# IannLiu/ReactRanker

Measured on AMD Instinct MI355X. Metric: queries/sec (lists scored+loss) ListMLE, higher is better.
Workload: dtype f32; 1 GPU; ListMLE 100k queries x 64 candidates (BASELINE.json configs[2]), 64-query steps, D-MPNN depth=3 hidden=300; preset=mle64, phase=train step: fwd + loss + bwd + grad all-reduce + Adam/NoamLR, candidates_per_query=64, pad_width_K=4, step_pool=6, parallelism=dp1

## Files before the change

include/reactranker_hip.h:

```cpp
#ifndef REACTRANKER_HIP_H
#define REACTRANKER_HIP_H

#include <stddef.h>
#include <stdint.h>

#ifdef __cplusplus
extern "C" {
#endif

typedef void* rr_stream_t;

typedef enum rr_status {
  RR_OK = 0,
  RR_ERR_ARG = -1,
  RR_ERR_ALIGN = -2,
  RR_ERR_LAUNCH = -3,
  RR_ERR_UNSUPPORTED = -4,
  RR_ERR_WORKSPACE = -5
} rr_status;

const char* rr_strerror(int status);
int rr_version(void);
void rr_abi_struct_sizes(size_t* linear_args, size_t* wgrad_args);
size_t rr_abi_gather_epi_size(void);
// ... 7 lines not shown
                             const int32_t* idx, int64_t n_out, int K, int H,
                             const float* row0_partial, int64_t n_partial, int64_t ld_partial,
                             float* out, int64_t ld_out, rr_stream_t stream);
int rr_gather_sum_amax_f32(const float* src, int64_t n_src, int64_t ld_src, const int32_t* idx, int64_t n_out, int K,
                           int H, const float* row0_partial, int64_t n_partial, int64_t ld_partial, float* out,
                           int64_t ld_out, float* amax_out, rr_stream_t stream);

int rr_gather_sum_masked_f32(const float* src, const float* mask, int64_t n_src, int64_t ld_src,
                             const int32_t* idx, int64_t n_out, int K, int H, float scale,
                             float* out, int64_t ld_out, rr_stream_t stream);
int rr_gather_sum_dropmask_f32(const float* src, int64_t n_src, int64_t ld_src, const float* y, int64_t ld_y,
                               const int32_t* idx, int64_t n_out, int K, int H, float drop_p, uint64_t drop_seed,
                               float scale, float* out, int64_t ld_out, rr_stream_t stream);

int rr_gather2_sum_dropmask_f32(const float* src, int64_t n_src, int64_t ld_src, const int32_t* in_idx, int64_t n_mid, int Ki,
                                const float* row0_partial, int64_t n_partial, int64_t ld_partial,
                                const float* y, int64_t ld_y, const int32_t* out_idx, int64_t n_out, int Ko, int H,
                                float drop_p, uint64_t drop_seed, float scale, float* out, int64_t ld_out,
                                rr_stream_t stream);

int rr_gather_sum_dropsrc_f32(const float* y, int64_t n_y, int64_t ld_y, const int32_t* map, int64_t n_map,
                              const int32_t* idx, int64_t n_out, int K, int H, float drop_p, uint64_t drop_seed,
                              float* out, int64_t ld_out, rr_stream_t stream);

#define RR_MAX_GATHER_SRCS 4
int rr_gather_sum_multi_f32(const float* const* srcs, int n_srcs, int64_t n_src, int64_t ld_src,
                            const int32_t* idx, int64_t n_out, int K, int H,
                            float* out, int64_t ld_out, rr_stream_t stream);

#define RR_MAX_GATHER_ADDS 15
typedef struct rr_gather_epi {
  const float* mask;        int64_t ld_mask;
  const uint8_t* mask_bits;
  float mask_scale;
  int n_adds;               int64_t ld_add;
  const float* adds[RR_MAX_GATHER_ADDS];
  float* amax_out;
} rr_gather_epi;
int rr_gather_sum_epi_f32(const float* src, int64_t n_src, int64_t ld_src,
                          const int32_t* idx, int64_t n_out, int K, int H,
                          const float* row0_partial, int64_t n_partial, int64_t ld_partial,
                          const rr_gather_epi* epi, float* out, int64_t ld_out, rr_stream_t stream);

int rr_gather_sum_csr_f32(const float* src, int64_t n_src, int64_t ld_src,
                          const int32_t* offsets, const int32_t* idx, int64_t n_out, int H,
                          float* out, int64_t ld_out, rr_stream_t stream);
// ... 558 lines not shown
```

reactranker_amd/_lib.py:

```python
from __future__ import annotations

import ctypes as C
import os

import torch

_HERE = os.path.dirname(os.path.abspath(__file__))
LIB_PATH = os.environ.get("RR_LIB_PATH") or os.path.join(_HERE, "csrc", "libreactranker_hip.so")

c_f32p = C.c_void_p
c_i32p = C.c_void_p
c_stream = C.c_void_p
i64 = C.c_int64
i32 = C.c_int
u64 = C.c_uint64
f32 = C.c_float


class LinearArgs(C.Structure):
    _fields_ = [
        ("M", i64), ("N", i32),
        ("a1", c_f32p), ("lda1", i64), ("k1", i32), ("a1_idx", c_i32p),
        ("a1_sub", c_f32p), ("lda1_sub", i64), ("a1_sub_idx", c_i32p),
        ("a2", c_f32p), ("lda2", i64), ("k2", i32),
# ... 134 lines not shown

_SIGS = {
    "rr_strerror": (C.c_char_p, [i32]),
    "rr_version": (i32, []),
    "rr_lds_opt_ins": (C.c_longlong, []),
    "rr_abi_struct_sizes": (None, [C.POINTER(C.c_size_t), C.POINTER(C.c_size_t)]),
    "rr_gather_sum_f32": (i32, [c_f32p, i64, i64, c_i32p, i64, i32, i32, c_f32p, i64, c_stream]),
    "rr_abi_gather_epi_size": (C.c_size_t, []),
    "rr_gather_sum_epi_f32": (i32, [c_f32p, i64, i64, c_i32p, i64, i32, i32, c_f32p, i64, i64, C.POINTER(GatherEpi), c_f32p, i64,
                                    c_stream]),
    "rr_segment_mean_bwd_masked_f32": (i32, [c_f32p, i64, c_i32p, c_i32p, i64, i32, i32, f32, u64, c_f32p, i64, C.c_void_p, f32,
                                             c_f32p, i64, c_stream]),
    "rr_segment_mean_bwd_masked_amax_f32": (i32, [c_f32p, i64, c_i32p, c_i32p, i64, i32, i32, f32, u64, c_f32p, i64, C.c_void_p, f32,
                                             c_f32p, i64, c_f32p, c_stream]),
    "rr_gather_sum_masked_f32": (i32, [c_f32p, c_f32p, i64, i64, c_i32p, i64, i32, i32, f32, c_f32p, i64, c_stream]),
    "rr_gather_sum_dropmask_f32": (i32, [c_f32p, i64, i64, c_f32p, i64, c_i32p, i64, i32, i32, f32, u64, f32, c_f32p, i64, c_stream]),
    "rr_gather2_sum_dropmask_f32": (i32, [c_f32p, i64, i64, c_i32p, i64, i32, c_f32p, i64, i64, c_f32p, i64, c_i32p, i64, i32, i32,
                                          f32, u64, f32, c_f32p, i64, c_stream]),
    "rr_gather_sum_dropsrc_f32": (i32, [c_f32p, i64, i64, c_i32p, i64, c_i32p, i64, i32, i32, f32, u64, c_f32p, i64, c_stream]),
    "rr_gather_sum_csr_f32": (i32, [c_f32p, i64, i64, c_i32p, c_i32p, i64, i32, c_f32p, i64, c_stream]),
    "rr_build_fbonds_f32": (i32, [c_f32p, i64, i64, i32, c_i32p, c_f32p, i64, i32, i64, c_f32p, i64, c_stream]),
    "rr_gather_diff_f32": (i32, [c_f32p, i64, i64, c_i32p, c_f32p, i64, i64, c_i32p, i64, i32, c_f32p, i64, c_stream]),
    "rr_gather_dropout_f32": (i32, [c_f32p, i64, i64, c_i32p, i64, i32, f32, u64, c_f32p, i64, c_stream]),
    "rr_gather_dropout_amax_f32": (i32, [c_f32p, i64, i64, c_i32p, i64, i32, f32, u64, c_f32p, i64, c_f32p, c_stream]),
    "rr_colsum_workspace_bytes": (C.c_size_t, [i64, i32]),
    "rr_weighted_colsum_f32": (i32, [c_f32p, i64, i64, c_f32p, i32, c_f32p, i32, C.c_void_p, C.c_size_t, c_stream]),
    "rr_linear_f32": (i32, [C.POINTER(LinearArgs), c_stream]),
    "rr_linear_colsum_rows": (i64, [i64]),
    "rr_linear_split_tail_launches": (i64, []),
    "rr_gather_sum_multi_f32": (i32, [C.POINTER(C.c_void_p), i32, i64, i64, c_i32p, i64, i32, i32, c_f32p, i64, c_stream]),
    "rr_gather_sum_padrow_f32": (i32, [c_f32p, i64, i64, c_i32p, i64, i32, i32, c_f32p, i64, i64, c_f32p, i64, c_stream]),
    "rr_gather_sum_amax_f32": (i32, [c_f32p, i64, i64, c_i32p, i64, i32, i32, c_f32p, i64, i64, c_f32p, i64, c_f32p, c_stream]),
    "rr_packed_weight_ld": (i64, [i32, i32]),
    "rr_mask_bits_row_bytes": (i64, [i32]),
    "rr_split_weight_bytes": (C.c_size_t, [i32, i32, i32]),
    "rr_pack_weight_f32": (i32, [c_f32p, i64, i32, i32, i32, i32, i32, c_f32p, c_stream]),
    "rr_pack_weights_f32": (i32, [C.c_void_p, i32, c_stream]),
    "rr_linear_wgrad_workspace_bytes": (C.c_size_t, [i64, i32, i32]),
    "rr_linear_wgrad_f32": (i32, [C.POINTER(WgradArgs), c_stream]),
    "rr_amax_f32": (i32, [c_f32p, i64, i32, i64, c_f32p, c_stream]),
    "rr_dropout_keep_host": (i32, [u64, u64, f32]),
    "rr_dropout_f32": (i32, [c_f32p, i64, f32, u64, c_f32p, c_stream]),
    "rr_relu_bwd_f32": (i32, [c_f32p, c_f32p, f32, c_f32p, c_f32p, i64, c_stream]),
    "rr_relu_bwd_sum_f32": (i32, [c_f32p, c_f32p, f32, C.POINTER(C.c_void_p), i32, c_f32p, i64, c_stream]),
    "rr_axpby_f32": (i32, [f32, c_f32p, f32, c_f32p, c_f32p, i64, c_stream]),
    "rr_head_fwd_f32": (i32, [c_f32p, i64, i32, i32, c_f32p, c_stream]),
# ... 218 lines not shown
```

reactranker_amd/csrc/gather.hip:

```cpp
#include "rr_common.h"
#include <initializer_list>

namespace {

template <int VEC> struct Vec;
template <> struct Vec<4> { using T = f32x4; };
template <> struct Vec<1> { using T = float; };

template <int VEC>
__device__ inline typename Vec<VEC>::T ld(const float* p) {
  return *reinterpret_cast<const typename Vec<VEC>::T*>(p);
}
template <int VEC>
__device__ inline void st(float* p, typename Vec<VEC>::T v) {
  *reinterpret_cast<typename Vec<VEC>::T*>(p) = v;
}

__device__ __attribute__((aligned(16))) const float gather_zero[4] = {0.f, 0.f, 0.f, 0.f};

template <int VEC>
__device__ __forceinline__ typename Vec<VEC>::T ld_row(const float* src, int64_t ld_src, int32_t j, int c) {
  return ld<VEC>(j >= 0 ? src + j * ld_src + c : gather_zero);
}

// ... 372 lines not shown
      for (int t = 0; t < Ko; ++t) {
        const int32_t j = orow[t];
        f32x4 inner = f32x4(0.0f);
        if (j >= 0) inner = gather_plain_sum<4>(A.src, A.ld_src, A.in_idx + static_cast<int64_t>(j) * Ki, Ki, c);
        acc = acc + dropmask_term(A, j, c, yv, inner);
      }
    }
    st<4>(A.out + r * A.ld_out + c, acc);
  }
}

struct DropSrc {
  const float* y;          int64_t ld_y;
  const int32_t* map;
  const int32_t* idx;      int64_t n_out; int K;
  int HV, H;
  uint32_t thr; float keep_scale; uint64_t seed;
  float* out;              int64_t ld_out;
};
__device__ __forceinline__ f32x4 dropsrc_term(const DropSrc& A, int32_t j, int c, f32x4 v) {
  if (A.thr != 0u) v = keep_scale4(v, A.seed, static_cast<uint64_t>(j < 0 ? 0 : j) * static_cast<uint64_t>(A.H) + static_cast<uint64_t>(c), A.thr, A.keep_scale);
  return v;
}
template <int KT>
__global__ void __launch_bounds__(256) gather_sum_dropsrc_kernel(const DropSrc A) {
  const int HV = A.HV, K = A.K;
  const int64_t total = A.n_out * HV;
#ifdef RR_GATHER_WALK
  if constexpr (KT > 0) {
    int64_t beg, end;
    gather_block_range(static_cast<int>(gridDim.x), total, &beg, &end);
    int64_t e = beg + threadIdx.x;
    if (e >= end) return;
    const int quo = 256 / HV, rem = 256 - quo * HV;
    int64_t r = e / HV;
    int q = static_cast<int>(e - r * HV);
    auto next = [&](int64_t& rr, int& qq) {
      rr += quo;
      qq += rem;
      if (qq >= HV) {
        qq -= HV;
        ++rr;
      }
    };
    auto maps = [&](const int32_t (&jj)[KT], int32_t (&mm)[KT]) {
#pragma unroll
      for (int k = 0; k < KT; ++k) mm[k] = A.map[jj[k] < 0 ? 0 : jj[k]];
    };
    int64_t r1 = r;
    int q1 = q;
    next(r1, q1);
    bool has1 = e + 256 < end;
    int32_t j[KT], m[KT], j1[KT], m1[KT], j2[KT];
#pragma unroll
    for (int k = 0; k < KT; ++k) j[k] = A.idx[r * KT + k];
#pragma unroll
    for (int k = 0; k < KT; ++k) j1[k] = A.idx[(has1 ? r1 : r) * KT + k];
    maps(j, m);
    while (true) {
      int64_t r2 = r1;
      int q2 = q1;
      next(r2, q2);
      const bool has2 = e + 512 < end;
#pragma unroll
      for (int k = 0; k < KT; ++k) j2[k] = A.idx[(has2 ? r2 : r) * KT + k];
      maps(j1, m1);
      const int c = q * 4;
      f32x4 v[KT];
#pragma unroll
      for (int k = 0; k < KT; ++k) v[k] = ld<4>(A.y + static_cast<int64_t>((j[k] < 0 || m[k] < 0) ? 0 : m[k]) * A.ld_y + c);
      f32x4 acc = f32x4(0.0f);
#pragma unroll
      for (int k = 0; k < KT; ++k) {
        f32x4 t = f32x4(0.0f);
        if (j[k] >= 0 && m[k] >= 0) t = dropsrc_term(A, j[k], c, v[k]);
        acc = acc + t;
      }
      st<4>(A.out + r * A.ld_out + c, acc);
      if (!has1) break;
      e += 256;
      r = r1;
      q = q1;
      r1 = r2;
      q1 = q2;
      has1 = has2;
#pragma unroll
      for (int k = 0; k < KT; ++k) {
        j[k] = j1[k];
        m[k] = m1[k];
        j1[k] = j2[k];
      }
    }
    return;
  }
#endif
  RR_GATHER_LOOP(e, static_cast<int>(gridDim.x), total) {
    const int64_t r = e / HV;
    const int c = static_cast<int>(e - r * HV) * 4;
    const f32x4 acc = gather_row_sum<f32x4>(
        A.idx + r * K, K,
        [&](int32_t j) { return ld_row<4>(A.y, A.ld_y, *(j >= 0 ? A.map + j : gather_none), c); },
        [&](int32_t j, f32x4 v) { return dropsrc_term(A, j, c, v); });
    st<4>(A.out + r * A.ld_out + c, acc);
  }
}

constexpr int GMAX = RR_MAX_GATHER_ADDS;
struct GatherEpi {
  const float* mask;   int64_t ld_mask;
  const uint8_t* bits; int64_t bits_row;
  float scale;
  int n_adds;          int64_t ld_add;
  const float* adds[GMAX];
  float* amax_out;
};

__device__ inline uint32_t epi_nibble(const uint8_t* bits, int64_t bits_row, int64_t r, int c) {
  const int blk = c / 304, cc = c - blk * 304;
  const uint32_t b = bits[r * bits_row + blk * 40 + ((cc & 15) >> 3) * 20 + (cc >> 4)];
  return (b >> (cc & 4)) & 0xFu;
}

template <int NADD>
struct EpiAux {
  uint32_t nib;
  f32x4 m;
  f32x4 a[NADD > 0 ? NADD : 1];
// ... 281 lines not shown
__global__ void __launch_bounds__(256) segment_mean_bwd_kernel(const float* __restrict__ dout, int64_t ld_dout,
                                                               const int32_t* __restrict__ a_scope,
                                                               const int32_t* __restrict__ atom2mol, int64_t n_atoms,
                                                               int H, int F, uint32_t thr, float keep_scale,
                                                               uint64_t seed, float* __restrict__ dx, int64_t ldx) {
  const int64_t total = n_atoms * H;
  const int64_t stride = static_cast<int64_t>(gridDim.x) * blockDim.x;
  const int W = H + F;
  for (int64_t e = static_cast<int64_t>(blockIdx.x) * blockDim.x + threadIdx.x; e < total; e += stride) {
    const int64_t a = e / H;
    const int c = static_cast<int>(e - a * H);
    const int32_t m = atom2mol[a];
    float v = 0.f;
    if (m >= 0) {
      const int32_t size = a_scope[2 * static_cast<int64_t>(m) + 1];
      v = dout[static_cast<int64_t>(m) * ld_dout + c] / static_cast<float>(size);
      if (thr != 0u)
        v = rr_keep(seed, static_cast<uint64_t>(m) * W + c, thr) ? v * keep_scale : 0.f;
    }
    dx[a * ldx + c] = v;
  }
}

__global__ void __launch_bounds__(256) segment_mean_bwd_vec_kernel(const float* __restrict__ dout, int64_t ld_dout,
                                                                   const int32_t* __restrict__ a_scope,
                                                                   const int32_t* __restrict__ atom2mol, int64_t n_atoms,
                                                                   int HV, int W, uint32_t thr, float keep_scale,
                                                                   uint64_t seed, float* __restrict__ dx, int64_t ldx,
                                                                   const float* __restrict__ mask, int64_t ld_mask,
                                                                   const uint8_t* __restrict__ mask_bits, int64_t bits_row,
                                                                   float mask_scale, float* __restrict__ amax_out) {
  const int64_t total = n_atoms * HV;
  const int64_t stride = static_cast<int64_t>(gridDim.x) * blockDim.x;
  float am = 0.f;
  for (int64_t e = static_cast<int64_t>(blockIdx.x) * blockDim.x + threadIdx.x; e < total; e += stride) {
    const int64_t a = e / HV;
    const int c = static_cast<int>(e - a * HV) * 4;
    const int32_t m = atom2mol[a];
    float4 v = make_float4(0.f, 0.f, 0.f, 0.f);
    if (m >= 0) {
      const float size = static_cast<float>(a_scope[2 * static_cast<int64_t>(m) + 1]);
      const float* d = dout + static_cast<int64_t>(m) * ld_dout + c;
      v = make_float4(d[0] / size, d[1] / size, d[2] / size, d[3] / size);
      if (thr != 0u) {
        const uint64_t i0 = static_cast<uint64_t>(m) * W + c;
        const uint32_t w0 = rr_hash_group(seed, i0 >> 2);
        const uint32_t w1 = (i0 & 3u) ? rr_hash_group(seed, (i0 >> 2) + 1) : w0;
        float* pv = &v.x;
#pragma unroll
        for (int k = 0; k < 4; ++k) {
          const uint64_t i = i0 + k;
          const uint32_t w = (i >> 2) == (i0 >> 2) ? w0 : w1;
          pv[k] = rr_hash_lane(w, static_cast<uint32_t>(i) & 3u) >= thr ? pv[k] * keep_scale : 0.f;
        }
      }
    }
    if (mask_bits != nullptr) v = mask_select(v, epi_nibble(mask_bits, bits_row, a, c), mask_scale);
    else if (mask != nullptr) v = mask_select(v, ld<4>(mask + a * ld_mask + c), mask_scale);
    *reinterpret_cast<float4*>(dx + a * ldx + c) = v;
    am = fmaxf(fmaxf(am, fmaxf(fabsf(v.x), fabsf(v.y))), fmaxf(fabsf(v.z), fabsf(v.w)));
  }
  amax_commit(am, amax_out);
}

bool rows_are_chunks(int H, std::initializer_list<int64_t> lds, std::initializer_list<const void*> ptrs) {
  bool ok = H % 4 == 0;
  for (const int64_t ld : lds) ok = ok && ld % 4 == 0;
  for (const void* p : ptrs) ok = ok && rr_aligned16(p);
  return ok;
}

#define RR_LAUNCH_ROWS(vec, kernel, n_out, H, pad_blocks, s, ...)                                       \
  do {                                                                                                  \
    if (vec) {                                                                                          \
      const int W = (H) / 4;                                                                            \
      kernel<4><<<rr_grid_for((n_out) * W, 256) + ((pad_blocks) ? W : 0), 256, 0, s>>>(__VA_ARGS__);    \
    } else {                                                                                            \
      const int W = (H);                                                                                \
      kernel<1><<<rr_grid_for((n_out) * W, 256) + ((pad_blocks) ? W : 0), 256, 0, s>>>(__VA_ARGS__);    \
    }                                                                                                   \
  } while (0)

}

extern "C" {

int rr_gather_sum_amax_f32(const float* src, int64_t n_src, int64_t ld_src, const int32_t* idx, int64_t n_out, int K,
                           int H, const float* row0_partial, int64_t n_partial, int64_t ld_partial, float* out,
                           int64_t ld_out, float* amax_out, rr_stream_t stream) {
  RR_CHECK_ARG(src && idx && out && n_src >= 0 && n_out >= 0 && K >= 1 && H >= 1 && ld_src >= H && ld_out >= H);
  RR_CHECK_ARG(!row0_partial || (n_out >= 1 && n_partial >= 0 && ld_partial >= H));
  if (n_out == 0) return RR_OK;
  hipStream_t s = static_cast<hipStream_t>(stream);
  bool vec = rows_are_chunks(H, {ld_src, ld_out}, {src, out});
  if (row0_partial) vec = vec && rows_are_chunks(H, {ld_partial}, {row0_partial});
  RR_LAUNCH_ROWS(vec, gather_sum_kernel, n_out, H, row0_partial != nullptr, s, src, ld_src, idx, n_out, K, W, out, ld_out,
                 row0_partial, n_partial, ld_partial, amax_out);
  return rr_launch_status();
}

int rr_gather_sum_f32(const float* src, int64_t n_src, int64_t ld_src, const int32_t* idx, int64_t n_out, int K,
                      int H, float* out, int64_t ld_out, rr_stream_t stream) {
  return rr_gather_sum_amax_f32(src, n_src, ld_src, idx, n_out, K, H, nullptr, 0, 0, out, ld_out, nullptr, stream);
}
// ... 132 lines not shown
  RR_CHECK_ARG(drop_p >= 0.f && drop_p < 1.f);
  if (!rows_are_chunks(H, {ld_y, ld_out}, {y, out})) return RR_ERR_ALIGN;
  if (n_out == 0) return RR_OK;
  DropSrc A;
  A.y = y; A.ld_y = ld_y; A.map = map; A.idx = idx; A.n_out = n_out; A.K = K; A.HV = H / 4; A.H = H;
  A.thr = rr_drop_threshold(drop_p); A.keep_scale = 1.0f / (1.0f - drop_p); A.seed = drop_seed; A.out = out; A.ld_out = ld_out;
  hipStream_t s = static_cast<hipStream_t>(stream);
  if (n_map == 0 || n_y == 0) {
    if (hipMemset2DAsync(out, static_cast<size_t>(ld_out) * sizeof(float), 0, static_cast<size_t>(H) * sizeof(float),
                         static_cast<size_t>(n_out), s) != hipSuccess) return RR_ERR_LAUNCH;
    return RR_OK;
  }
  const int grid = rr_grid_for(n_out * A.HV, 256);
  switch (K) {
    case 1: gather_sum_dropsrc_kernel<1><<<grid, 256, 0, s>>>(A); break;
    case 2: gather_sum_dropsrc_kernel<2><<<grid, 256, 0, s>>>(A); break;
    case 3: gather_sum_dropsrc_kernel<3><<<grid, 256, 0, s>>>(A); break;
    case 4: gather_sum_dropsrc_kernel<4><<<grid, 256, 0, s>>>(A); break;
    default: gather_sum_dropsrc_kernel<0><<<grid, 256, 0, s>>>(A); break;
  }
  return rr_launch_status();
}

int rr_gather_sum_csr_f32(const float* src, int64_t n_src, int64_t ld_src, const int32_t* offsets, const int32_t* idx,
                          int64_t n_out, int H, float* out, int64_t ld_out, rr_stream_t stream) {
  RR_CHECK_ARG(src && offsets && out && n_src >= 0 && n_out >= 0 && H >= 1 && ld_src >= H && ld_out >= H);
  if (n_out == 0) return RR_OK;
  hipStream_t s = static_cast<hipStream_t>(stream);
  const bool vec = rows_are_chunks(H, {ld_src, ld_out}, {src, out});
  RR_LAUNCH_ROWS(vec, gather_sum_csr_kernel, n_out, H, false, s, src, ld_src, offsets, idx, n_out, W, out, ld_out);
  return rr_launch_status();
}

int rr_gather_diff_f32(const float* a, int64_t n_a, int64_t ld_a, const int32_t* ia, const float* m, int64_t n_m,
                       int64_t ld_m, const int32_t* im, int64_t n_out, int H, float* out, int64_t ld_out,
                       rr_stream_t stream) {
  RR_CHECK_ARG(a && ia && m && im && out && n_a >= 0 && n_m >= 0 && n_out >= 0 && H >= 1 && ld_a >= H &&
               ld_m >= H && ld_out >= H);
  if (n_out == 0) return RR_OK;
  hipStream_t s = static_cast<hipStream_t>(stream);
  const bool vec = rows_are_chunks(H, {ld_a, ld_m, ld_out}, {a, m, out});
  RR_LAUNCH_ROWS(vec, gather_diff_kernel, n_out, H, false, s, a, ld_a, ia, m, ld_m, im, n_out, W, out, ld_out);
  return rr_launch_status();
}

int rr_gather_dropout_f32(const float* src, int64_t n_src, int64_t ld_src, const int32_t* idx, int64_t n_out, int H,
// ... 69 lines not shown
                                                                         1.0f / (1.0f - drop_p), drop_seed, out,
                                                                         ld_out);
  return rr_launch_status();
}

int rr_segment_mean_bwd_masked_f32(const float* dout, int64_t ld_dout, const int32_t* a_scope, const int32_t* atom2mol,
                                   int64_t n_atoms, int H, int F, float drop_p, uint64_t drop_seed, const float* mask,
                                   int64_t ld_mask, const uint8_t* mask_bits, float mask_scale, float* dx, int64_t ldx,
                                   rr_stream_t stream) {
  return rr_segment_mean_bwd_masked_amax_f32(dout, ld_dout, a_scope, atom2mol, n_atoms, H, F, drop_p, drop_seed, mask, ld_mask,
                                             mask_bits, mask_scale, dx, ldx, nullptr, stream);
}

int rr_segment_mean_bwd_masked_amax_f32(const float* dout, int64_t ld_dout, const int32_t* a_scope, const int32_t* atom2mol,
                                        int64_t n_atoms, int H, int F, float drop_p, uint64_t drop_seed, const float* mask,
                                        int64_t ld_mask, const uint8_t* mask_bits, float mask_scale, float* dx, int64_t ldx,
                                        float* amax_out, rr_stream_t stream) {
  RR_CHECK_ARG(dout && a_scope && atom2mol && dx && n_atoms >= 0 && H >= 1 && F >= 0 && ld_dout >= H && ldx >= H);
  RR_CHECK_ARG(drop_p >= 0.f && drop_p < 1.f);
  RR_CHECK_ARG((mask || mask_bits) && (!mask || ld_mask >= H));
  if (n_atoms == 0) return RR_OK;
  if (!rows_are_chunks(H, {ldx}, {dx})) return RR_ERR_ALIGN;
  if (!mask_bits && !rows_are_chunks(H, {ld_mask}, {mask})) return RR_ERR_ALIGN;
  segment_mean_bwd_vec_kernel<<<rr_grid_for(n_atoms * (H / 4), 256), 256, 0, static_cast<hipStream_t>(stream)>>>(
      dout, ld_dout, a_scope, atom2mol, n_atoms, H / 4, H + F, rr_drop_threshold(drop_p), 1.0f / (1.0f - drop_p), drop_seed,
      dx, ldx, mask_bits ? nullptr : mask, ld_mask, mask_bits, rr_mask_bits_row_bytes(H), mask_scale, amax_out);
  return rr_launch_status();
}

int rr_segment_mean_bwd_f32(const float* dout, int64_t ld_dout, const int32_t* a_scope, const int32_t* atom2mol,
                            int64_t n_atoms, int H, int F, float drop_p, uint64_t drop_seed, float* dx, int64_t ldx,
                            rr_stream_t stream) {
  RR_CHECK_ARG(dout && a_scope && atom2mol && dx && n_atoms >= 0 && H >= 1 && F >= 0 && ld_dout >= H && ldx >= H);
  RR_CHECK_ARG(drop_p >= 0.f && drop_p < 1.f);
  if (n_atoms == 0) return RR_OK;
  hipStream_t s = static_cast<hipStream_t>(stream);
  const uint32_t thr = rr_drop_threshold(drop_p);
  if (rows_are_chunks(H, {ldx}, {dx})) {
    segment_mean_bwd_vec_kernel<<<rr_grid_for(n_atoms * (H / 4), 256), 256, 0, s>>>(
        dout, ld_dout, a_scope, atom2mol, n_atoms, H / 4, H + F, thr, 1.0f / (1.0f - drop_p), drop_seed, dx, ldx,
        nullptr, 0, nullptr, 0, 1.0f, nullptr);
  } else {
    segment_mean_bwd_kernel<<<rr_grid_for(n_atoms * H, 256), 256, 0, s>>>(dout, ld_dout, a_scope, atom2mol, n_atoms, H,
                                                                          F, thr, 1.0f / (1.0f - drop_p), drop_seed, dx,
                                                                          ldx);
  }
  return rr_launch_status();
}

}
```

reactranker_amd/csrc/plan.hip:

```cpp
#include <stdio.h>
#include <stdlib.h>
#include <string.h>

#include <mutex>
#include <vector>

#include "rr_common.h"

namespace {

constexpr int ATOM_FDIM = 61;

inline uint64_t site_seed(uint64_t seed, uint64_t site) {
  return seed * 0x9E3779B97F4A7C15ull + site * 0xD1B54A32D192ED03ull;
}
inline int64_t r4(int64_t n) { return (n + 3) / 4 * 4; }

struct Arena {
  char* base;
  size_t off, cap;
  bool overflow;
  float* f(int64_t rows, int64_t cols) {
    const size_t bytes = (static_cast<size_t>(rows < 1 ? 1 : rows) * static_cast<size_t>(cols) * sizeof(float) + 255) & ~size_t(255);
    const size_t at = off;
// ... 63 lines not shown
  float* alloc(int64_t rows, int64_t cols) {
    float* p = ar.f(rows, cols);
    if (f16 && p != nullptr && !ar.overflow) reg(p, rows, cols, cols);
    return p;
  }
  void reg(const float* p, int64_t rows, int64_t cols, int64_t ld) {
    if (!tracked(p) || find(p) != nullptr) return;
    if (ntr == MAX_TENSORS) { fail(RR_ERR_UNSUPPORTED); return; }
    tr[ntr].p = p; tr[ntr].rows = rows; tr[ntr].cols = cols; tr[ntr].ld = ld; tr[ntr].amax = nullptr;
    ++ntr;
  }
  bool claim_slot(TensorRec& r) {
    if (namax == MAX_AMAX) { fail(RR_ERR_UNSUPPORTED); return false; }
    r.amax = amax_base + static_cast<size_t>(namax++) * RR_AMAX_FLOATS;
    return true;
  }
  Streams s = {nullptr, nullptr, nullptr};
  bool use_side = false, use_aux = false, aux_bwd = false;
  bool train = false;
  bool ffn_chain = true;
  bool timing = false;
  bool gather_multi = false;
  bool prefix_fuse = false;
  bool wgrad_early = false;
  bool tail_pass = false;
  bool side_joined = false;
  hipStream_t cur = nullptr;
  bool split = false;
  rr_pack_desc pq[RR_MAX_PACK] = {};
  int npq = 0;
  void fail(int st) { if (status == RR_OK && st != RR_OK) status = st; }
};

Ctx make_ctx(int flags, void* workspace, size_t workspace_bytes, bool launch) {
  Ctx c;
  c.launch = launch;
  c.ar.base = static_cast<char*>(workspace);
  c.ar.cap = workspace_bytes;
  c.use_side = (flags & RR_PLAN_NO_SIDE_STREAM) == 0;
  c.use_aux = (flags & RR_PLAN_NO_AUX_STREAM) == 0;
  c.split = (flags & RR_PLAN_F32_GEMM) == 0;
  c.f16 = c.split && (flags & RR_PLAN_F16X2_GEMM) != 0;
  c.aux_bwd = (flags & RR_PLAN_AUX_BACKWARD) != 0;
  c.train = (flags & RR_PLAN_TRAIN) != 0;
  c.ffn_chain = (flags & RR_PLAN_NO_FFN_CHAIN) == 0 && !getenv("RR_NO_FFN_CHAIN");
  c.timing = (flags & RR_PLAN_TIME) != 0;
  c.gather_multi = !getenv("RR_NO_GATHER_MULTI");
  c.prefix_fuse = !getenv("RR_NO_PREFIX_FUSE");
  c.wgrad_early = (flags & RR_PLAN_WGRAD_EARLY) != 0 || getenv("RR_WGRAD_EARLY") != nullptr;
  return c;
}

#define RR_TRY(ctx, expr)                                                                         \
  do {                                                                                            \
    if ((ctx).launch && (ctx).status == RR_OK) {                                                  \
      (ctx).fail(expr);                                                                           \
      if ((ctx).status != RR_OK && getenv("RR_PLAN_DEBUG"))                                       \
        fprintf(stderr, "[rr plan] status %d at plan.hip:%d: %s\n", (ctx).status, __LINE__, #expr); \
    }                                                                                             \
  } while (0)

const float* amax_of(Ctx& c, const float* t, hipStream_t st) {
  if (!c.tracked(t)) return nullptr;
  TensorRec* r = c.find(t);
  if (r == nullptr) {
    if (getenv("RR_PLAN_DEBUG")) fprintf(stderr, "[rr plan] amax_of: unknown tensor %p\n", static_cast<const void*>(t));
    c.fail(RR_ERR_ARG);
    return nullptr;
  }
  if (r->amax == nullptr) {
    if (!c.claim_slot(*r)) return nullptr;
// ... 242 lines not shown
  const float* npad;
  const int32_t *b2a, *b2revb;
  const float* x2; int64_t ld_x2; int k2;
  Operand message(const float* a_msg, const float* msg, int H) const {
    return b2a != nullptr ? minus(a_msg, b2a, msg, b2revb, H) : plain(a_msg, H, H);
  }
};
Rel bonds(const rr_graph& g) { return {g.nA, g.nB, g.a2b, g.K, g.b2t, 1, g.b2b_t, g.Kb, g.npad_b, g.b2a, g.b2revb, nullptr, 0, 0}; }
Rel atoms(const rr_graph& g, int FB) { return {g.nA, g.nA, g.a2a, g.K, g.a2a_t, g.K, g.a2a_t, g.K, g.npad, nullptr, nullptr, g.fb_sum, g.ld_fbs, FB}; }

void wi_forward(Ctx& c, int64_t rows, int H, const Operand& in, const Packed& W, const float* bias, float p, uint64_t seed,
                float*& inp, float*& msg, uint8_t** bits, hipStream_t st) {
  inp = c.alloc(rows, H);
  msg = c.alloc(rows, H);
  rr_linear_args a = LA(rows, H);
  set_a1(a, in);
  set_w(a, W); a.bias = bias; a.act = RR_ACT_RELU; a.drop_p = p; a.drop_seed = seed;
  a.c_pre = inp; a.ld_pre = H;
  set_out(c, a, msg, rows, H, W, bits);
  lin(c, a, st);
}

void wh_forward(Ctx& c, const Rel& R, int H, const Packed& W, const float* bias, const float* msg, float*& a_msg, float*& out,
                uint8_t** bits, const float* inp, const int32_t* inp_idx, float p, uint64_t seed, hipStream_t st) {
  a_msg = c.alloc(R.nA, H);
  gather_sum(c, msg, R.rows, H, R.fwd, R.nA, R.K, H, a_msg, H, st);
  out = c.alloc(R.rows, H);
  rr_linear_args a = LA(R.rows, H);
  set_a1(a, R.message(a_msg, msg, H)); a.a2 = R.x2; a.lda2 = R.ld_x2; a.k2 = R.k2;
  set_w(a, W); a.bias = bias; a.residual = inp; a.ldr = H; a.residual_idx = inp_idx; a.act = RR_ACT_RELU;
  a.drop_p = p; a.drop_seed = seed;
  set_out(c, a, out, R.rows, H, W, bits);
  lin(c, a, st);
}

void wo_forward(Ctx& c, const Rel& R, int H, const Operand& first, const Packed& W, const float* bias, float p, uint64_t seed,
                const float* msg, MpSaved& S, hipStream_t st) {
  S.a_last = c.alloc(R.nA, H);
  gather_sum(c, msg, R.rows, H, R.fwd, R.nA, R.K, H, S.a_last, H, st);
  S.out = c.alloc(R.nA, H);
  rr_linear_args a = LA(R.nA, H);
  set_a1(a, first); a.a2 = S.a_last; a.lda2 = H; a.k2 = H;
  set_w(a, W); a.bias = bias; a.act = RR_ACT_RELU; a.drop_p = p; a.drop_seed = seed;
  set_out(c, a, S.out, R.nA, H, W, &S.bits_out);
  lin(c, a, st);
}

void mpn_forward(Ctx& c, const rr_model& m, const rr_graph& g, const PackedW& pk, float p, uint64_t seed, MpSaved& S,
                 hipStream_t st) {
  const int H = m.H, depth = m.depth;
  const Rel R = bonds(g);
  float* inp;
  wi_forward(c, g.nB, H, plain(g.f_bonds, g.ld_fb, m.bond_fdim), pk.enc_wi, m.enc_wi.b, 0.f, 0, inp, S.msgs[0], &S.bits[0], st);
  for (int it = 0; it < depth - 1; ++it)
    wh_forward(c, R, H, pk.enc_wh, m.enc_wh.b, S.msgs[it], S.amsgs[it], S.msgs[it + 1], &S.bits[it + 1], inp, nullptr, p,
               site_seed(seed, it), st);
  wo_forward(c, R, H, plain(g.f_atoms, g.ld_fa, m.atom_fdim), pk.enc_wo, m.enc_wo.b, p, site_seed(seed, 1000), S.msgs[depth - 1], S,
             st);
}

void mpn_forward_shared(Ctx& c, const rr_model& m, const rr_graph& gu, const rr_graph& g, const int32_t* bmap,
                        const PackedW& pk, float p, uint64_t seed, MpSaved& S, hipStream_t st) {
  const int H = m.H, depth = m.depth;
  const Rel R = bonds(g);
  float* inp_u;
  wi_forward(c, gu.nB, H, plain(gu.f_bonds, gu.ld_fb, m.bond_fdim), pk.enc_wi, m.enc_wi.b, 0.f, 0, inp_u, S.msg0_u, nullptr, st);
  wh_forward(c, bonds(gu), H, pk.enc_wh, m.enc_wh.b, S.msg0_u, S.a0_u, S.z1_u, nullptr, inp_u, nullptr, 0.f, 0, st);
  S.msgs[0] = nullptr;
  S.msgs[1] = c.alloc(g.nB, H);
  S.seed0 = site_seed(seed, 0);
  RR_TRY(c, rr_gather_dropout_amax_f32(S.z1_u, gu.nB, H, bmap, g.nB, H, p, S.seed0, S.msgs[1], H, amax_claim(c, S.msgs[1]), st));
  for (int it = 1; it < depth - 1; ++it)
    wh_forward(c, R, H, pk.enc_wh, m.enc_wh.b, S.msgs[it], S.amsgs[it], S.msgs[it + 1], &S.bits[it + 1], inp_u, bmap, p,
               site_seed(seed, it), st);
  wo_forward(c, R, H, plain(g.f_atoms, g.ld_fa, m.atom_fdim), pk.enc_wo, m.enc_wo.b, p, site_seed(seed, 1000), S.msgs[depth - 1], S,
             st);
}

void mpndiff_forward(Ctx& c, const rr_model& m, const rr_graph& g, const PackedW& pk, float p, uint64_t seed, const float* x,
                     const float* x_sub, const int32_t* x_sub_idx, const float* feat, int F, uint64_t out_seed, MpSaved& S,
                     hipStream_t st) {
  const int H = m.H, depth = m.diff_depth;
  const Rel R = atoms(g, m.bond_fdim);
  const Operand feats = minus(x, nullptr, x_sub, x_sub_idx, H);
  float* inp;
  wi_forward(c, g.nA, H, feats, pk.dif_wi, m.dif_wi.b, depth == 0 ? p : 0.f, site_seed(seed, 2000), inp, S.msgs[0], &S.bits[0],
             st);
  if (depth > 0) {
    for (int it = 0; it < depth - 1; ++it)
      wh_forward(c, R, H, pk.dif_wh, m.dif_wh.b, S.msgs[it], S.amsgs[it], S.msgs[it + 1], &S.bits[it + 1], inp, nullptr, p,
                 site_seed(seed, 2001 + it), st);
    wo_forward(c, R, H, feats, pk.dif_wo, m.dif_wo.b, p, site_seed(seed, 3000), S.msgs[depth - 1], S, st);
  } else {
    S.a_last = nullptr;
    S.out = S.msgs[0];
  }
  S.ld_vecs = r4(H + F);
// ... 603 lines not shown
```

reactranker_amd/functions.py:

```python
from __future__ import annotations

import os

import ctypes as C
from typing import List, Optional

import torch

from . import _lib
from ._lib import LinearArgs, WgradArgs, check, lib, ptr, stream

ACT_NONE, ACT_RELU = 0, 1
ATOM_FDIM, BOND_FDIM = 61, 22
FBOND = ATOM_FDIM + BOND_FDIM

HEADS = {
    "evidential_with_softplus": 6, "gauss_regression_with_softplus": 4, "gaussian_with_softplus": 4,
    "listnetdis_lognorm_with_softplus": 5, "evidential_ranking": 3, "listnet_with_softplus": 1,
    "listnet_with_uncertainty": 2, "evidential": 2,
}


class Profiler:
    enabled = False
# ... 115 lines not shown
    n_mid, Ki = in_idx.shape
    n_out, Ko = out_idx.shape
    if out is None:
        out = _new(src, n_out, H)
    assert y.shape[0] == n_out
    with _Timed("gather2_sum_dropmask_kernel", 0, 4 * (src.shape[0] * H + 2 * n_out * H + n_out * Ko + n_mid * Ki)):
        check(lib().rr_gather2_sum_dropmask_f32(ptr(src), src.shape[0], _ld(src), ptr(in_idx), n_mid, Ki, ptr(row0_partial),
                                                0 if row0_partial is None else row0_partial.shape[0], _ld(row0_partial),
                                                ptr(y), _ld(y), ptr(out_idx), n_out, Ko, H, float(p),
                                                int(seed) & 0xFFFFFFFFFFFFFFFF, float(scale), ptr(out), _ld(out), stream()),
              "rr_gather2_sum_dropmask_f32")
    return out


def gather_sum_dropsrc(y, copies, idx, H: int, p: float, seed: int, out=None):
    n_out, K = (idx.shape[0], idx.shape[1]) if idx.dim() == 2 else (idx.shape[0], 1)
    if out is None:
        out = _new(y, n_out, H)
    with _Timed("gather_sum_dropsrc_kernel", 0, 4 * (y.shape[0] * H + n_out * H + n_out * K + copies.shape[0])):
        check(lib().rr_gather_sum_dropsrc_f32(ptr(y), y.shape[0], _ld(y), ptr(copies), copies.shape[0], ptr(idx), n_out, K, H,
                                              float(p), int(seed) & 0xFFFFFFFFFFFFFFFF, ptr(out), _ld(out), stream()),
              "rr_gather_sum_dropsrc_f32")
    return out


MAX_GATHER_SRCS = _lib.RR_MAX_GATHER_SRCS


def gather_sum_multi(srcs, idx, H: int, out=None):
    srcs = list(srcs)
    limit = MAX_GATHER_SRCS if (H % 4 == 0 and not os.environ.get("RR_NO_GATHER_MULTI")) else 1
    while len(srcs) > limit:
        srcs = [axpby(1.0, srcs[0], 1.0, srcs[1])] + srcs[2:]
    if len(srcs) == 1:
        return gather_sum(srcs[0], idx, H, out=out)
    n_out, K = idx.shape
    if out is None:
        out = _new(srcs[0], n_out, H)
    assert all(t.shape == srcs[0].shape and t.stride(0) == srcs[0].stride(0) for t in srcs)
    arr = (C.c_void_p * len(srcs))(*[t.data_ptr() for t in srcs])
    with _Timed("gather_sum_multi_kernel", 0, 4 * (len(srcs) * srcs[0].shape[0] * H + n_out * H + n_out * K)):
        check(lib().rr_gather_sum_multi_f32(arr, len(srcs), srcs[0].shape[0], _ld(srcs[0]), ptr(idx), n_out, K, H, ptr(out),
                                            _ld(out), stream()), "rr_gather_sum_multi_f32")
    return out


# ... 1113 lines not shown
```

Before: 13410 queries/s.

## Fuse first-layer dropout copy with atom gather-sum and walk molecules in readout backward

Adds a fused kernel that applies dropout to the first message layer, stores the per-bond rows and sums them into atom aggregates in one pass. Extra blocks handle bonds not listed in any atom's index. The encoder forward uses it when depth>=3 and skips the separate gather_sum in the first wh_forward step. Separately, the segment-mean backward (readout adjoint) now walks runs of consecutive atoms and reuses the per-molecule scaled gradient chunk instead of recomputing it per atom. Both aim to cut memory traffic and kernel launches, at the cost of more complex kernels and a redundant ownership scan for unlisted rows.

```diff
diff --git a/include/reactranker_hip.h b/include/reactranker_hip.h
--- a/include/reactranker_hip.h
+++ b/include/reactranker_hip.h
@@ -53,6 +53,11 @@
 int rr_gather_sum_dropsrc_f32(const float* y, int64_t n_y, int64_t ld_y, const int32_t* map, int64_t n_map,
                               const int32_t* idx, int64_t n_out, int K, int H, float drop_p, uint64_t drop_seed,
                               float* out, int64_t ld_out, rr_stream_t stream);
+
+int rr_gather_dropout_sum_f32(const float* y, int64_t n_y, int64_t ld_y, const int32_t* map, int64_t n_rows,
+                              const int32_t* idx, int64_t n_out, int K, const int32_t* owner, int H, float drop_p,
+                              uint64_t drop_seed, float* rows, int64_t ld_rows, float* rows_amax, float* out, int64_t ld_out,
+                              rr_stream_t stream);
 
 #define RR_MAX_GATHER_SRCS 4
 int rr_gather_sum_multi_f32(const float* const* srcs, int n_srcs, int64_t n_src, int64_t ld_src,
diff --git a/reactranker_amd/_lib.py b/reactranker_amd/_lib.py
--- a/reactranker_amd/_lib.py
+++ b/reactranker_amd/_lib.py
@@ -180,6 +180,8 @@
     "rr_build_fbonds_f32": (i32, [c_f32p, i64, i64, i32, c_i32p, c_f32p, i64, i32, i64, c_f32p, i64, c_stream]),
     "rr_gather_diff_f32": (i32, [c_f32p, i64, i64, c_i32p, c_f32p, i64, i64, c_i32p, i64, i32, c_f32p, i64, c_stream]),
     "rr_gather_dropout_f32": (i32, [c_f32p, i64, i64, c_i32p, i64, i32, f32, u64, c_f32p, i64, c_stream]),
+    "rr_gather_dropout_sum_f32": (i32, [c_f32p, i64, i64, c_i32p, i64, c_i32p, i64, i32, c_i32p, i32, f32, u64, c_f32p, i64, c_f32p,
+                                        c_f32p, i64, c_stream]),
     "rr_gather_dropout_amax_f32": (i32, [c_f32p, i64, i64, c_i32p, i64, i32, f32, u64, c_f32p, i64, c_f32p, c_stream]),
     "rr_colsum_workspace_bytes": (C.c_size_t, [i64, i32]),
     "rr_weighted_colsum_f32": (i32, [c_f32p, i64, i64, c_f32p, i32, c_f32p, i32, C.c_void_p, C.c_size_t, c_stream]),
diff --git a/reactranker_amd/csrc/gather.hip b/reactranker_amd/csrc/gather.hip
--- a/reactranker_amd/csrc/gather.hip
+++ b/reactranker_amd/csrc/gather.hip
@@ -1,4 +1,5 @@
 #include "rr_common.h"
+#include <cstdlib>
 #include <initializer_list>
 
 namespace {
@@ -418,16 +419,28 @@
   if (A.thr != 0u) v = keep_scale4(v, A.seed, static_cast<uint64_t>(j < 0 ? 0 : j) * static_cast<uint64_t>(A.H) + static_cast<uint64_t>(c), A.thr, A.keep_scale);
   return v;
 }
-template <int KT>
-__global__ void __launch_bounds__(256) gather_sum_dropsrc_kernel(const DropSrc A) {
+struct DropStore {
+  float* rows;             int64_t ld_rows; int64_t n_rows;
+  const int32_t* owner;
+  float* amax_out;
+};
+template <int KT, bool STORE>
+__device__ __forceinline__ float dropsrc_walk(const DropSrc& A, const DropStore& X, int gblocks) {
   const int HV = A.HV, K = A.K;
   const int64_t total = A.n_out * HV;
+  float am = 0.f;
+  auto keep = [&](int32_t j, int c, f32x4 t) {
+    if (j > 0) {
+      st<4>(X.rows + static_cast<int64_t>(j) * X.ld_rows + c, t);
+      am = amax_fold(am, t);
+    }
+  };
 #ifdef RR_GATHER_WALK
   if constexpr (KT > 0) {
     int64_t beg, end;
-    gather_block_range(static_cast<int>(gridDim.x), total, &beg, &end);
+    gather_block_range(gblocks, total, &beg, &end);
     int64_t e = beg + threadIdx.x;
-    if (e >= end) return;
+    if (e >= end) return am;
     const int quo = 256 / HV, rem = 256 - quo * HV;
     int64_t r = e / HV;
     int q = static_cast<int>(e - r * HV);
@@ -470,6 +483,7 @@
       for (int k = 0; k < KT; ++k) {
         f32x4 t = f32x4(0.0f);
         if (j[k] >= 0 && m[k] >= 0) t = dropsrc_term(A, j[k], c, v[k]);
+        if constexpr (STORE) keep(j[k], c, t);
         acc = acc + t;
       }
       st<4>(A.out + r * A.ld_out + c, acc);
@@ -487,18 +501,52 @@
         j1[k] = j2[k];
       }
     }
-    return;
+    return am;
   }
 #endif
-  RR_GATHER_LOOP(e, static_cast<int>(gridDim.x), total) {
+  RR_GATHER_LOOP(e, gblocks, total) {
     const int64_t r = e / HV;
     const int c = static_cast<int>(e - r * HV) * 4;
     const f32x4 acc = gather_row_sum<f32x4>(
         A.idx + r * K, K,
         [&](int32_t j) { return ld_row<4>(A.y, A.ld_y, *(j >= 0 ? A.map + j : gather_none), c); },
-        [&](int32_t j, f32x4 v) { return dropsrc_term(A, j, c, v); });
+        [&](int32_t j, f32x4 v) {
+          const f32x4 t = dropsrc_term(A, j, c, v);
+          if constexpr (STORE) keep(j, c, t);
+          return t;
+        });
     st<4>(A.out + r * A.ld_out + c, acc);
   }
+  return am;
+}
+template <int KT>
+__global__ void __launch_bounds__(256) gather_sum_dropsrc_kernel(const DropSrc A) {
+  dropsrc_walk<KT, false>(A, DropStore{}, static_cast<int>(gridDim.x));
+}
+
+template <int KT>
+__global__ void __launch_bounds__(256) gather_dropout_sum_kernel(const DropSrc A, const DropStore X, int gblocks) {
+  float am = 0.f;
+  if (static_cast<int>(blockIdx.x) < gblocks) {
+    am = dropsrc_walk<KT, true>(A, X, gblocks);
+  } else {
+    const int64_t b = (static_cast<int64_t>(blockIdx.x) - gblocks) * 256 + threadIdx.x;
+    if (b < X.n_rows) {
+      bool listed = false;
+      const int64_t a = b > 0 ? X.owner[b] : -1;
+      if (a >= 0 && a < A.n_out)
+        for (int k = 0; k < A.K; ++k) listed = listed || A.idx[a * A.K + k] == b;
+      if (!listed) {
+        const int32_t m = A.map[b];
+        for (int c = 0; c < A.H; c += 4) {
+          const f32x4 t = dropsrc_term(A, static_cast<int32_t>(b), c, ld_row<4>(A.y, A.ld_y, m, c));
+          st<4>(X.rows + b * X.ld_rows + c, t);
+          am = amax_fold(am, t);
+        }
+      }
+    }
+  }
+  amax_commit(am, X.amax_out);
 }
 
 constexpr int GMAX = RR_MAX_GATHER_ADDS;
@@ -826,6 +874,27 @@
   }
 }
 
+__device__ __forceinline__ float4 readout_adjoint_chunk(const float* __restrict__ dout, int64_t ld_dout,
+                                                        const int32_t* __restrict__ a_scope, int32_t m, int c, int W,
+                                                        uint32_t thr, float keep_scale, uint64_t seed) {
+  const float size = static_cast<float>(a_scope[2 * static_cast<int64_t>(m) + 1]);
+  const float* d = dout + static_cast<int64_t>(m) * ld_dout + c;
+  float4 v = make_float4(d[0] / size, d[1] / size, d[2] / size, d[3] / size);
+  if (thr != 0u) {
+    const uint64_t i0 = static_cast<uint64_t>(m) * W + c;
+    const uint32_t w0 = rr_hash_group(seed, i0 >> 2);
+    const uint32_t w1 = (i0 & 3u) ? rr_hash_group(seed, (i0 >> 2) + 1) : w0;
+    float* pv = &v.x;
+#pragma unroll
+    for (int k = 0; k < 4; ++k) {
+      const uint64_t i = i0 + k;
+      const uint32_t w = (i >> 2) == (i0 >> 2) ? w0 : w1;
+      pv[k] = rr_hash_lane(w, static_cast<uint32_t>(i) & 3u) >= thr ? pv[k] * keep_scale : 0.f;
+    }
+  }
+  return v;
+}
+
 __global__ void __launch_bounds__(256) segment_mean_bwd_vec_kernel(const float* __restrict__ dout, int64_t ld_dout,
                                                                    const int32_t* __restrict__ a_scope,
                                                                    const int32_t* __restrict__ atom2mol, int64_t n_atoms,
@@ -842,27 +911,66 @@
     const int c = static_cast<int>(e - a * HV) * 4;
     const int32_t m = atom2mol[a];
     float4 v = make_float4(0.f, 0.f, 0.f, 0.f);
-    if (m >= 0) {
-      const float size = static_cast<float>(a_scope[2 * static_cast<int64_t>(m) + 1]);
-      const float* d = dout + static_cast<int64_t>(m) * ld_dout + c;
-      v = make_float4(d[0] / size, d[1] / size, d[2] / size, d[3] / size);
-      if (thr != 0u) {
-        const uint64_t i0 = static_cast<uint64_t>(m) * W + c;
-        const uint32_t w0 = rr_hash_group(seed, i0 >> 2);
-        const uint32_t w1 = (i0 & 3u) ? rr_hash_group(seed, (i0 >> 2) + 1) : w0;
-        float* pv = &v.x;
-#pragma unroll
-        for (int k = 0; k < 4; ++k) {
-          const uint64_t i = i0 + k;
-          const uint32_t w = (i >> 2) == (i0 >> 2) ? w0 : w1;
-          pv[k] = rr_hash_lane(w, static_cast<uint32_t>(i) & 3u) >= thr ? pv[k] * keep_scale : 0.f;
-        }
-      }
-    }
+    if (m >= 0) v = readout_adjoint_chunk(dout, ld_dout, a_scope, m, c, W, thr, keep_scale, seed);
     if (mask_bits != nullptr) v = mask_select(v, epi_nibble(mask_bits, bits_row, a, c), mask_scale);
     else if (mask != nullptr) v = mask_select(v, ld<4>(mask + a * ld_mask + c), mask_scale);
     *reinterpret_cast<float4*>(dx + a * ldx + c) = v;
     am = fmaxf(fmaxf(am, fmaxf(fabsf(v.x), fabsf(v.y))), fmaxf(fabsf(v.z), fabsf(v.w)));
+  }
+  amax_commit(am, amax_out);
+}
+
+template <int MASK>
+__global__ void __launch_bounds__(256) segment_mean_bwd_walk_kernel(const float* __restrict__ dout, int64_t ld_dout,
+                                                                    const int32_t* __restrict__ a_scope,
+                                                                    const int32_t* __restrict__ atom2mol, int64_t n_atoms,
+                                                                    int HV, int G, int L, int W, uint32_t thr,
+                                                                    float keep_scale, uint64_t seed, float* __restrict__ dx,
+                                                                    int64_t ldx, const float* __restrict__ mask,
+                                                                    int64_t ld_mask, const uint8_t* __restrict__ mask_bits,
+                                                                    int64_t bits_row, float mask_scale,
+                                                                    float* __restrict__ amax_out) {
+  const int items = G * HV;
+  const int64_t first = static_cast<int64_t>(blockIdx.x) * G * L;
+  float am = 0.f;
+  for (int i = threadIdx.x; i < items; i += 256) {
+    const int g = i / HV;
+    const int c = (i - g * HV) * 4;
+    const int64_t a0 = first + static_cast<int64_t>(g) * L;
+    if (a0 >= n_atoms) continue;
+    const int n = n_atoms - a0 < L ? static_cast<int>(n_atoms - a0) : L;
+    int32_t mol[4], mol_next[4];
+#pragma unroll
+    for (int j = 0; j < 4; ++j) mol_next[j] = atom2mol[a0 + (j < n ? j : 0)];
+    int32_t cur = -1;
+    float4 base = make_float4(0.f, 0.f, 0.f, 0.f);
+    for (int k0 = 0; k0 < n; k0 += 4) {
+      uint32_t nib[4];
+      f32x4 mk[4];
+#pragma unroll
+      for (int j = 0; j < 4; ++j) {
+        mol[j] = mol_next[j];
+        mol_next[j] = atom2mol[a0 + (k0 + 4 + j < n ? k0 + 4 + j : 0)];
+        const int64_t a = a0 + (k0 + j < n ? k0 + j : 0);
+        if constexpr (MASK == 2) nib[j] = epi_nibble(mask_bits, bits_row, a, c);
+        if constexpr (MASK == 1) mk[j] = ld<4>(mask + a * ld_mask + c);
+      }
+#pragma unroll
+      for (int j = 0; j < 4; ++j) {
+        if (k0 + j >= n) break;
+        const int32_t m = mol[j];
+        if (m != cur) {
+          cur = m;
+          base = make_float4(0.f, 0.f, 0.f, 0.f);
+          if (m >= 0) base = readout_adjoint_chunk(dout, ld_dout, a_scope, m, c, W, thr, keep_scale, seed);
+        }
+        float4 v = base;
+        if constexpr (MASK == 2) v = mask_select(v, nib[j], mask_scale);
+        if constexpr (MASK == 1) v = mask_select(v, mk[j], mask_scale);
+        *reinterpret_cast<float4*>(dx + (a0 + k0 + j) * ldx + c) = v;
+        am = fmaxf(fmaxf(am, fmaxf(fabsf(v.x), fabsf(v.y))), fmaxf(fabsf(v.z), fabsf(v.w)));
+      }
+    }
   }
   amax_commit(am, amax_out);
 }
@@ -884,6 +992,32 @@
       kernel<1><<<rr_grid_for((n_out) * W, 256) + ((pad_blocks) ? W : 0), 256, 0, s>>>(__VA_ARGS__);    \
     }                                                                                                   \
   } while (0)
+
+void launch_readout_adjoint_vec(const float* dout, int64_t ld_dout, const int32_t* a_scope, const int32_t* atom2mol,
+                                int64_t n_atoms, int H, int F, uint32_t thr, float keep_scale, uint64_t seed, float* dx,
+                                int64_t ldx, const float* mask, int64_t ld_mask, const uint8_t* mask_bits, float mask_scale,
+                                float* amax_out, hipStream_t s) {
+  const int HV = H / 4, W = H + F;
+  const int64_t bits_row = mask_bits ? rr_mask_bits_row_bytes(H) : 0;
+  if (getenv("RR_NO_MOLECULE_WALK")) {
+    segment_mean_bwd_vec_kernel<<<rr_grid_for(n_atoms * HV, 256), 256, 0, s>>>(
+        dout, ld_dout, a_scope, atom2mol, n_atoms, HV, W, thr, keep_scale, seed, dx, ldx, mask, ld_mask, mask_bits, bits_row,
+        mask_scale, amax_out);
+    return;
+  }
+  const int L = 8;
+  const int G = HV < 256 ? 256 / HV : 1;
+  const int64_t per_block = static_cast<int64_t>(G) * L;
+  const unsigned grid = static_cast<unsigned>((n_atoms + per_block - 1) / per_block);
+#define RR_READOUT_WALK(MASK)                                                                                             \
+  segment_mean_bwd_walk_kernel<MASK><<<grid, 256, 0, s>>>(dout, ld_dout, a_scope, atom2mol, n_atoms, HV, G, L, W, thr,    \
+                                                          keep_scale, seed, dx, ldx, mask, ld_mask, mask_bits, bits_row,   \
+                                                          mask_scale, amax_out)
+  if (mask_bits != nullptr) RR_READOUT_WALK(2);
+  else if (mask != nullptr) RR_READOUT_WALK(1);
+  else RR_READOUT_WALK(0);
+#undef RR_READOUT_WALK
+}
 
 }
 
@@ -1062,6 +1196,31 @@
   return rr_launch_status();
 }
 
+int rr_gather_dropout_sum_f32(const float* y, int64_t n_y, int64_t ld_y, const int32_t* map, int64_t n_rows, const int32_t* idx,
+                              int64_t n_out, int K, const int32_t* owner, int H, float drop_p, uint64_t drop_seed, float* rows,
+                              int64_t ld_rows, float* rows_amax, float* out, int64_t ld_out, rr_stream_t stream) {
+  RR_CHECK_ARG(y && map && idx && owner && rows && out && n_y >= 1 && n_rows >= 1 && n_rows < INT32_MAX && n_out >= 0 && K >= 1 &&
+               H >= 1 && ld_y >= H && ld_rows >= H && ld_out >= H);
+  RR_CHECK_ARG(drop_p >= 0.f && drop_p < 1.f);
+  if (!rows_are_chunks(H, {ld_y, ld_rows, ld_out}, {y, rows, out})) return RR_ERR_ALIGN;
+  DropSrc A;
+  A.y = y; A.ld_y = ld_y; A.map = map; A.idx = idx; A.n_out = n_out; A.K = K; A.HV = H / 4; A.H = H;
+  A.thr = rr_drop_threshold(drop_p); A.keep_scale = 1.0f / (1.0f - drop_p); A.seed = drop_seed; A.out = out; A.ld_out = ld_out;
+  DropStore X;
+  X.rows = rows; X.ld_rows = ld_rows; X.n_rows = n_rows; X.owner = owner; X.amax_out = rows_amax;
+  hipStream_t s = static_cast<hipStream_t>(stream);
+  const int gblocks = rr_grid_for(n_out * A.HV, 256);
+  const int grid = gblocks + static_cast<int>((n_rows + 255) / 256);
+  switch (K) {
+    case 1: gather_dropout_sum_kernel<1><<<grid, 256, 0, s>>>(A, X, gblocks); break;
+    case 2: gather_dropout_sum_kernel<2><<<grid, 256, 0, s>>>(A, X, gblocks); break;
+    case 3: gather_dropout_sum_kernel<3><<<grid, 256, 0, s>>>(A, X, gblocks); break;
+    case 4: gather_dropout_sum_kernel<4><<<grid, 256, 0, s>>>(A, X, gblocks); break;
+    default: gather_dropout_sum_kernel<0><<<grid, 256, 0, s>>>(A, X, gblocks); break;
+  }
+  return rr_launch_status();
+}
+
 int rr_gather_sum_csr_f32(const float* src, int64_t n_src, int64_t ld_src, const int32_t* offsets, const int32_t* idx,
                           int64_t n_out, int H, float* out, int64_t ld_out, rr_stream_t stream) {
   RR_CHECK_ARG(src && offsets && out && n_src >= 0 && n_out >= 0 && H >= 1 && ld_src >= H && ld_out >= H);
@@ -1177,9 +1336,9 @@
   if (n_atoms == 0) return RR_OK;
   if (!rows_are_chunks(H, {ldx}, {dx})) return RR_ERR_ALIGN;
   if (!mask_bits && !rows_are_chunks(H, {ld_mask}, {mask})) return RR_ERR_ALIGN;
-  segment_mean_bwd_vec_kernel<<<rr_grid_for(n_atoms * (H / 4), 256), 256, 0, static_cast<hipStream_t>(stream)>>>(
-      dout, ld_dout, a_scope, atom2mol, n_atoms, H / 4, H + F, rr_drop_threshold(drop_p), 1.0f / (1.0f - drop_p), drop_seed,
-      dx, ldx, mask_bits ? nullptr : mask, ld_mask, mask_bits, rr_mask_bits_row_bytes(H), mask_scale, amax_out);
+  launch_readout_adjoint_vec(dout, ld_dout, a_scope, atom2mol, n_atoms, H, F, rr_drop_threshold(drop_p), 1.0f / (1.0f - drop_p),
+                             drop_seed, dx, ldx, mask_bits ? nullptr : mask, ld_mask, mask_bits, mask_scale, amax_out,
+                             static_cast<hipStream_t>(stream));
   return rr_launch_status();
 }
 
@@ -1192,9 +1351,8 @@
   hipStream_t s = static_cast<hipStream_t>(stream);
   const uint32_t thr = rr_drop_threshold(drop_p);
   if (rows_are_chunks(H, {ldx}, {dx})) {
-    segment_mean_bwd_vec_kernel<<<rr_grid_for(n_atoms * (H / 4), 256), 256, 0, s>>>(
-        dout, ld_dout, a_scope, atom2mol, n_atoms, H / 4, H + F, thr, 1.0f / (1.0f - drop_p), drop_seed, dx, ldx,
-        nullptr, 0, nullptr, 0, 1.0f, nullptr);
+    launch_readout_adjoint_vec(dout, ld_dout, a_scope, atom2mol, n_atoms, H, F, thr, 1.0f / (1.0f - drop_p), drop_seed, dx, ldx,
+                               nullptr, 0, nullptr, 1.0f, nullptr, s);
   } else {
     segment_mean_bwd_kernel<<<rr_grid_for(n_atoms * H, 256), 256, 0, s>>>(dout, ld_dout, a_scope, atom2mol, n_atoms, H,
                                                                           F, thr, 1.0f / (1.0f - drop_p), drop_seed, dx,
diff --git a/reactranker_amd/csrc/plan.hip b/reactranker_amd/csrc/plan.hip
--- a/reactranker_amd/csrc/plan.hip
+++ b/reactranker_amd/csrc/plan.hip
@@ -109,6 +109,7 @@
   bool timing = false;
   bool gather_multi = false;
   bool prefix_fuse = false;
+  bool copy_walk = false;
   bool wgrad_early = false;
   bool tail_pass = false;
   bool side_joined = false;
@@ -134,6 +135,7 @@
   c.timing = (flags & RR_PLAN_TIME) != 0;
   c.gather_multi = !getenv("RR_NO_GATHER_MULTI");
   c.prefix_fuse = !getenv("RR_NO_PREFIX_FUSE");
+  c.copy_walk = !getenv("RR_NO_COPY_WALK");
   c.wgrad_early = (flags & RR_PLAN_WGRAD_EARLY) != 0 || getenv("RR_WGRAD_EARLY") != nullptr;
   return c;
 }
@@ -422,9 +424,12 @@
 }
 
 void wh_forward(Ctx& c, const Rel& R, int H, const Packed& W, const float* bias, const float* msg, float*& a_msg, float*& out,
-                uint8_t** bits, const float* inp, const int32_t* inp_idx, float p, uint64_t seed, hipStream_t st) {
-  a_msg = c.alloc(R.nA, H);
-  gather_sum(c, msg, R.rows, H, R.fwd, R.nA, R.K, H, a_msg, H, st);
+                uint8_t** bits, const float* inp, const int32_t* inp_idx, float p, uint64_t seed, hipStream_t st,
+                bool have_a_msg = false) {
+  if (!have_a_msg) {
+    a_msg = c.alloc(R.nA, H);
+    gather_sum(c, msg, R.rows, H, R.fwd, R.nA, R.K, H, a_msg, H, st);
+  }
   out = c.alloc(R.rows, H);
   rr_linear_args a = LA(R.rows, H);
   set_a1(a, R.message(a_msg, msg, H)); a.a2 = R.x2; a.lda2 = R.ld_x2; a.k2 = R.k2;
@@ -469,10 +474,21 @@
   S.msgs[0] = nullptr;
   S.msgs[1] = c.alloc(g.nB, H);
   S.seed0 = site_seed(seed, 0);
-  RR_TRY(c, rr_gather_dropout_amax_f32(S.z1_u, gu.nB, H, bmap, g.nB, H, p, S.seed0, S.msgs[1], H, amax_claim(c, S.msgs[1]), st));
+  const bool walk = c.copy_walk && !c.f16 && H % 4 == 0 && depth >= 3;
+  if (walk) {
+    S.amsgs[1] = c.alloc(g.nA, H);
+    rr_plan_timing ti;
+    memset(&ti, 0, sizeof(ti));
+    ti.kind = 1; ti.M = g.nA; ti.n_src = g.nB; ti.N = H; ti.k1 = g.K;
+    Timed t(c, st, ti, g.nA >= 8192);
+    RR_TRY(c, rr_gather_dropout_sum_f32(S.z1_u, gu.nB, H, bmap, g.nB, g.a2b, g.nA, g.K, g.b2t, H, p, S.seed0, S.msgs[1], H, nullptr,
+                                        S.amsgs[1], H, st));
+  } else {
+    RR_TRY(c, rr_gather_dropout_amax_f32(S.z1_u, gu.nB, H, bmap, g.nB, H, p, S.seed0, S.msgs[1], H, amax_claim(c, S.msgs[1]), st));
+  }
   for (int it = 1; it < depth - 1; ++it)
     wh_forward(c, R, H, pk.enc_wh, m.enc_wh.b, S.msgs[it], S.amsgs[it], S.msgs[it + 1], &S.bits[it + 1], inp_u, bmap, p,
-               site_seed(seed, it), st);
+               site_seed(seed, it), st, walk && it == 1);
   wo_forward(c, R, H, plain(g.f_atoms, g.ld_fa, m.atom_fdim), pk.enc_wo, m.enc_wo.b, p, site_seed(seed, 1000), S.msgs[depth - 1], S,
              st);
 }
diff --git a/reactranker_amd/functions.py b/reactranker_amd/functions.py
--- a/reactranker_amd/functions.py
+++ b/reactranker_amd/functions.py
@@ -161,6 +161,19 @@
                                               float(p), int(seed) & 0xFFFFFFFFFFFFFFFF, ptr(out), _ld(out), stream()),
               "rr_gather_sum_dropsrc_f32")
     return out
+
+
+def gather_dropout_sum(y, copies, idx, owner, H: int, p: float, seed: int, rows=None, out=None, rows_amax=None):
+    n_out, K = idx.shape
+    if rows is None:
+        rows = _new(y, copies.shape[0], H)
+    if out is None:
+        out = _new(y, n_out, H)
+    with _Timed("gather_dropout_sum_kernel", 0, 4 * (y.shape[0] * H + copies.shape[0] * H + n_out * H + n_out * K + 2 * copies.shape[0])):
+        check(lib().rr_gather_dropout_sum_f32(ptr(y), y.shape[0], _ld(y), ptr(copies), copies.shape[0], ptr(idx), n_out, K, ptr(owner),
+                                              H, float(p), int(seed) & 0xFFFFFFFFFFFFFFFF, ptr(rows), _ld(rows), ptr(rows_amax),
+                                              ptr(out), _ld(out), stream()), "rr_gather_dropout_sum_f32")
+    return rows, out
 
 
 MAX_GATHER_SRCS = _lib.RR_MAX_GATHER_SRCS
```

Result: no change. 13330 queries/s (-0.6%).
